# ahmetumutdurmus/zaremba

Measured on NVIDIA H100. Metric: tokens/sec (and valid perplexity) Large-LSTM 1500h at 1/2/4/8 H100 vs ref CPU, higher is better.
Workload: dtype f16 operands, f32 accumulate/state

## Files before the change

zaremba_b200/csrc/common.cuh:

```cuda
#pragma once
#include <cuda_runtime.h>
#include <cuda_fp16.h>
#include <stdint.h>
#include <stdio.h>
#include <atomic>

#include "../../include/zaremba_b200.h"

namespace zrb {

void set_error(const char* fmt, ...);
extern std::atomic<int64_t> g_launches;
extern std::atomic<int> g_live_tc_ctx[64];
inline void count_launch(int n = 1) { g_launches.fetch_add(n, std::memory_order_relaxed); }

#define ZRB_CUDA(call)                                                                   \
    do {                                                                                 \
        cudaError_t e_ = (call);                                                         \
        if (e_ != cudaSuccess) {                                                         \
            zrb::set_error("%s:%d %s -> %s", __FILE__, __LINE__, #call,                  \
                           cudaGetErrorString(e_));                                      \
            return ZRB_E_CUDA;                                                           \
        }                                                                                \
    } while (0)
// ... 105 lines not shown
    for (int i = 0; i < 4; ++i)
        if ((r.v[i] >> 8) >= m.thresh) bits |= 1u << i;
    return bits;
}

__device__ inline uint64_t mask_elem(const MaskSrc& m, uint64_t e) { return m.period ? e % m.period : e; }

__device__ inline float mask_mul1_at(const MaskSrc& m, uint64_t e, uint64_t n_total) {
    if (!m.active) return 1.f;
    uint32_t bits = mask_keep4(m, e >> 2, n_total);
    return ((bits >> (e & 3)) & 1u) ? m.scale : 0.f;
}

__device__ inline void mask_mul4_at(const MaskSrc& m, uint64_t e0, float out[4]) {
    if (!m.active) {
        out[0] = out[1] = out[2] = out[3] = 1.f;
        return;
    }
    const uint32_t sh = (uint32_t)(e0 & 3);
    uint32_t bits = mask_keep4(m, e0 >> 2, ~0ull) >> sh;
    if (sh) bits |= mask_keep4(m, (e0 >> 2) + 1, ~0ull) << (4 - sh);
#pragma unroll
    for (int i = 0; i < 4; ++i) out[i] = ((bits >> i) & 1u) ? m.scale : 0.f;
}

__device__ inline float mask_mul1(const MaskSrc& m, uint64_t e, uint64_t n_total) {
    if (!m.active) return 1.f;
    return mask_mul1_at(m, mask_elem(m, e), n_total);
}

__device__ inline float sigmoidf_(float z) { return 1.f / (1.f + expf(-z)); }

__device__ __forceinline__ float sgd_elem(float p, float g, float lr) { return p - lr * g; }

template <bool RMS>
__device__ __forceinline__ float dyneval_elem(float p, float g, float tg, float r, float lr, float lam, float eps,
                                              float rbar) {
    const float d = __fsub_rn(tg, p);
    const float u = RMS ? __fdiv_rn(g, __fadd_rn(r, eps)) : g;
    const float a = fminf(1.f, RMS ? __fdiv_rn(__fmul_rn(lam, r), rbar) : lam);
    return __fadd_rn(p, __fmaf_rn(a, d, -__fmul_rn(lr, u)));
}

struct DynArgs {
    float lr, lam, eps;
    const float* rbar;
};

__device__ inline float warp_sum(float v) {
#pragma unroll
    for (int o = 16; o > 0; o >>= 1) v += __shfl_xor_sync(0xffffffffu, v, o);
    return v;
}
__device__ inline float warp_max(float v) {
#pragma unroll
    for (int o = 16; o > 0; o >>= 1) v = fmaxf(v, __shfl_xor_sync(0xffffffffu, v, o));
    return v;
}

}
```

zaremba_b200/csrc/engine_tc.cu:

```cuda
#include "engine.h"
#include <stdlib.h>
#include <string.h>

#include "tc_kernels.h"

struct GridBarrier {
    unsigned int* word = nullptr;
    unsigned int base = 0;
    template <typename Launch>
    int claim(int T, int nCTA, cudaStream_t s, Launch&& launch) {
        const unsigned int arrivals = (unsigned int)T * (unsigned int)nCTA;
        if (base > 0xF0000000u - arrivals) {
            ZRB_CUDA(cudaMemsetAsync(word, 0, sizeof(unsigned int), s));
            base = 0;
        }
        ZRB_TRY(launch(word, base));
        base += arrivals;
        return ZRB_OK;
    }
};

struct zrb_tc_state {
    int Xp[ZRB_MAX_LAYERS + 1] = {}, G4p[ZRB_MAX_LAYERS] = {}, Vp = 0;
    int device = 0;
// ... 624 lines not shown
    const RecPlan& bplan = t->bplan[0];
    if (!c->layer_fwd_ok) {
        set_error("zrb_lstm_layer_bwd without a preceding zrb_lstm_layer_fwd");
        return ZRB_E_STATE;
    }
    MaskSrc m = make_mask_src(nullptr, 0, 0, 0, 0.f, 0);
    ZRB_TRY(t->bwd_bar.claim(T, bplan.nCTA, s, [&](unsigned int* word, unsigned int base) {
        return lstm_rec_bwd(bplan, tc_watchdog(c), t->w_img_b[0], t->g_img, dy, c->gates[0], c->cst[0], c->c0s[0], t->dG_h,
                            word, base, T, B, H, G4p, m, m, s, nullptr, db_ih, db_hh, c->resident_flag, ++c->resident_seq, c->dG);
    }));
    const float inv = 1.f / kGradScale;
    if (dx) ZRB_TRY(gemm_f16_tc(t->dG_h, G4p, 0, t->w_ih_h[0], Hp, 1, dx, H, N, H, 4 * H, inv, nullptr, 0, s));
    ZRB_TRY(gemm_f16_tc(t->dG_h, G4p, 1, t->x_h[0], Hp, 1, dw_ih, H, 4 * H, H, N, inv, nullptr, 0, s, nullptr, nullptr, false,
                        t->hprev_h[0], dw_hh, nullptr));
    c->layer_fwd_ok = false;
    return ZRB_OK;
}

int tc_rec_trace(zrb_ctx* c, long long* h_out, int max_entries) {
    if (!c->tc || !c->tc->trace) { set_error("set ZRB_REC_TRACE=1 before creating the context"); return ZRB_E_STATE; }
    int n = 2 * (8 + c->cfg.max_seq * 8);
    if (n > max_entries) n = max_entries;
    ZRB_CUDA(cudaDeviceSynchronize());
    ZRB_CUDA(cudaMemcpy(h_out, c->tc->trace, (size_t)n * sizeof(long long), cudaMemcpyDeviceToHost));
    return n;
}

int tc_update(zrb_ctx* c, const zrb_params* p, const TensorList& tl, float lr, float max_norm, float* norm_out,
              const AvgStep* avg, cudaStream_t s) {
    zrb_tc_state* t = c->tc;
    const int E = c->width[0], V = c->cfg.vocab;
    ZRB_TRY(tc_flush_updates(c, s));
    ProfScope ps(c, ZRB_PROF_CLIP_SGD, s);
    if (!tc_streams_aligned(tl, avg ? avg->a : nullptr)) {
        if (avg) {
            ZRB_TRY(grad_norm(tl, max_norm, c->partials, c->scalars, norm_out, s));
            ZRB_TRY(sgd_avg_apply(tl, avg->a, lr, c->scalars, c->keep_clipped, avg->mu, avg->first, s));
        } else {
            ZRB_TRY(clip_sgd(tl, lr, max_norm, c->partials, c->scalars, norm_out, c->keep_clipped, s));
        }
        c->weights_version++;
        return ZRB_OK;
    }
    const bool rows_only = !c->tied && c->emb_sparse && c->emb_prev_grad == tl.g[0] && c->emb_prev_n > 0;
    const bool gemm_norm = t->wg_ok && t->wg_key == tl.g[tc_matrices(c).fc_w().i];
    TensorList rest = tc_without_matrices(c, tl);
    if (rows_only) rest.n[0] = 0;
    TensorList dense = gemm_norm ? rest : tl;
    if (rows_only) dense.n[0] = 0;
    if (c->tied && gemm_norm) {
        ZRB_TRY(grad_norm(dense, max_norm, c->partials, c->scalars, norm_out, s, true, t->wg_slots));
    } else if (rows_only) {
        ZRB_TRY(embed_first_table(c->emb_prev_ids, c->emb_first, c->emb_prev_n, V, s));
        ZRB_TRY(embed_rows_sumsq(tl.g[0], c->emb_prev_ids, c->emb_first, c->emb_prev_n, E, V,
                                 c->partials + norm_partials_base(), kNormExtra, s));
        ZRB_TRY(grad_norm(dense, max_norm, c->partials, c->scalars, norm_out, s, true, gemm_norm ? t->wg_slots : 0));
        ZRB_TRY(embed_rows_update(tl.p[0], tl.g[0], c->emb_prev_ids, c->emb_first, c->emb_prev_n, E, V, lr, c->scalars,
                                  c->keep_clipped, s));
        if (avg) {
            TensorList e{};
            e.p[0] = tl.p[0]; e.n[0] = tl.n[0]; e.count = 1;
            ZRB_TRY(avg_apply(e, avg->a, avg->mu, avg->first, s));
        }
    } else {
        ZRB_TRY(grad_norm(tl, max_norm, c->partials, c->scalars, norm_out, s));
    }
    const bool lazy = c->lazy_update && t->persistent() && pdl_beside_rec(c);
    if (lazy) {
        t->upd_tl = tl;
        t->upd_lr = lr;
        t->upd_avg_on = avg != nullptr;
        if (avg) t->upd_avg = *avg;
    }
    for (const WeightMatrix& m : tc_matrices(c)) {
        if (lazy && m.item >= 1) t->upd_pending |= 1u << m.item;
        else ZRB_TRY(tc_update_matrix(c, m, tl, lr, avg, false, s));
    }
    if (avg) ZRB_TRY(sgd_avg_apply(rest, avg->a, lr, c->scalars, c->keep_clipped, avg->mu, avg->first, s));
    else ZRB_TRY(sgd_apply(rest, lr, c->scalars, c->keep_clipped, s));
    tc_images_current(c, p);
    return ZRB_OK;
}

int tc_dyneval_update(zrb_ctx* c, const zrb_params* p, const TensorList& tl, float* const* tg, float* const* r,
                      const DynArgs& a, cudaStream_t s) {
    ZRB_TRY(tc_flush_updates(c, s));
    ProfScope ps(c, ZRB_PROF_CLIP_SGD, s);
    if (!tc_streams_aligned(tl, tg, r)) {
        ZRB_TRY(dyneval_apply(tl, tg, r, a, s));
        c->weights_version++;
        return ZRB_OK;
    }
    for (const WeightMatrix& m : tc_matrices(c))
        ZRB_TRY(update_pack_dyn(tl.p[m.i], tl.g[m.i], tg[m.i], r ? r[m.i] : nullptr, m.rows, m.cols, a,
                                tc_images(c, m, {}), s));
    ZRB_TRY(dyneval_apply(tc_without_matrices(c, tl), tg, r, a, s));
    tc_images_current(c, p);
    return ZRB_OK;
}

int tc_swap_average(zrb_ctx* c, const zrb_params* p, const TensorList& tl, float* const* a, cudaStream_t s) {
    ZRB_TRY(tc_flush_updates(c, s));
    ProfScope ps(c, ZRB_PROF_PACK, s);
    if (!tc_streams_aligned(tl, a)) {
        ZRB_TRY(swap_apply(tl, a, s));
        c->weights_version++;
        return ZRB_OK;
    }
    for (const WeightMatrix& m : tc_matrices(c)) ZRB_TRY(swap_pack(tl.p[m.i], a[m.i], m.rows, m.cols, tc_images(c, m, {}), s));
// ... 7 lines not shown
```

zaremba_b200/csrc/kernels.h:

```cpp
#pragma once
#include "common.cuh"

namespace zrb {

int embed_dropout_fwd(const float* W, const int64_t* idx, float* out, __half* out_h, int64_t ld_h,
                      int N, int H, int V, MaskSrc m, MaskSrc em, cudaStream_t s, const float* pend_g = nullptr,
                      float lr = 0.f, const float* scalars = nullptr);
int embed_dropout_bwd(const float* dA, const int64_t* idx, float* dW, int N, int H, int V, MaskSrc m, MaskSrc em,
                      cudaStream_t s);
int lstm_cell_fwd(float* pre, const float* c_prev, float* c_out, float* h_raw, float* y_out, float* h_rec,
                  int B, int H, int64_t elem_off, int64_t n_total, MaskSrc m, MaskSrc rm, cudaStream_t s);
int lstm_cell_bwd(const float* dy_post, const float* dh_rec, float* dc, const float* gates, const float* c_t,
                  const float* c_prev, float* dG, int B, int H, int64_t elem_off, int64_t n_total, MaskSrc m,
                  MaskSrc rm, cudaStream_t s, const float* r = nullptr);
int activation_reg(const float* h, float* r, double* partial, float* out, int T, int B, int H, MaskSrc m, float alpha,
                   float beta, cudaStream_t s);
constexpr int kActRegBlocks = 264;
int dropout_copy(const float* x, float* y, int64_t n, MaskSrc m, cudaStream_t s);
constexpr int kWeightDropBlocks = 264;
int weight_drop(const float* x, float* y, int64_t n, MaskSrc m, float* sumsq, cudaStream_t s);
int add_bias2(float* C, const float* b1, const float* b2, int N, int M, cudaStream_t s);
int add_bias1(float* C, const float* b1, int N, int M, cudaStream_t s);
int colsum(const float* A, float* out, float* out2, int N, int M, cudaStream_t s);
int softmax_nll(const float* scores, const int64_t* y, int N, int V, int B, float* row_loss, float* loss,
                float* dscores, float* tgt_prob, cudaStream_t s, __half* ds_h = nullptr, int64_t ld_s = 0,
                float h_scale = 1.f);
int embed_rows(const float* dA, const int64_t* idx, float* rows, int N, int H, int V, MaskSrc m, MaskSrc em,
               cudaStream_t s);
int embed_scatter_rows(const int64_t* ids, const float* rows, float* dW, int n_rows, int H, int V, int* first,
                       long long* acc, cudaStream_t s, bool add = false, float* sumsq = nullptr, int nblocks = 0);
int embed_zero_rows(float* dW, const int64_t* ids, int n, int H, int V, cudaStream_t s);
int embed_first_table(const int64_t* ids, int* first, int n, int V, cudaStream_t s);
int embed_rows_sumsq(const float* dW, const int64_t* ids, const int* first, int n, int H, int V, float* partial,
                     int nblocks, cudaStream_t s);
int embed_rows_update(float* W, float* dW, const int64_t* ids, const int* first, int n, int H, int V, float lr,
                      const float* scalars, bool write_g, cudaStream_t s);
int dropout_mask_bytes(MaskSrc m, int64_t n, uint8_t* out, cudaStream_t s);

struct TensorList {
    float* p[16];
    float* g[16];
    int64_t n[16];
    int count;
};
constexpr int kNormGemm = 16384;
constexpr int kNormExtra = 1024;
int norm_partials_base();
int grad_norm(const TensorList& tl, float max_norm, float* partials, float* scalars, float* norm_out,
              cudaStream_t s, bool extra_used = false, int n_gemm = 0);
int sgd_apply(const TensorList& tl, float lr, const float* scalars, bool write_g, cudaStream_t s);
int clip_sgd(const TensorList& tl, float lr, float max_norm, float* partials, float* scalars, float* norm_out,
             bool write_g, cudaStream_t s);
int dyneval_apply(const TensorList& tl, float* const* tg, float* const* r, const DynArgs& a, cudaStream_t s);
int sq_accumulate(const TensorList& tl, cudaStream_t s);
constexpr int kStatsPartials = 2048;
int stats_finish(const TensorList& tl, int64_t windows, double* partials, float* rbar, cudaStream_t s);

struct AvgStep {
    float* a[16];
    float mu;
    bool first;
};
int sgd_avg_apply(const TensorList& tl, float* const* a, float lr, const float* scalars, bool write_g, float mu,
                  bool first, cudaStream_t s);
int avg_apply(const TensorList& tl, float* const* a, float mu, bool first, cudaStream_t s);
int swap_apply(const TensorList& tl, float* const* a, cudaStream_t s);

int sample_check(const zrb_sampling* cfg, int B, int V);
int sample_rows(const float* scores, int64_t ld, int B, int V, const zrb_sampling* cfg, uint64_t pos, int64_t* tokens,
                float* logprobs, cudaStream_t s);

struct BeamCand {
    float cand, logp;
    uint32_t flat;
};
struct LayerWidths {
    int h[ZRB_MAX_LAYERS];
};
int beam_check(int B, int K, int V, int eos);
int beam_step(const float* scores, int64_t ld, int B, int K_in, int K, int V, const float* cum_in, const int64_t* tok_in,
              int eos, BeamCand* cands, int64_t* tokens, int32_t* parents, float* cum_out, float* logprobs,
              const zrb_states* src, const zrb_states* dst, int L, const LayerWidths& w, cudaStream_t s);
int beam_backtrack(const int64_t* step_tok, const int32_t* step_par, const float* step_lp, const float* cum, int n_new,
                   int BK, int K, int64_t* tokens, float* logprobs, float* scores, cudaStream_t s);

int gemm_f32(const float* A, const float* B, float* C, int M, int N, int K, int transA, int transB, float alpha,
             float beta, cudaStream_t s);

}
```

zaremba_b200/csrc/optim.cu:

```cuda
#include "kernels.h"

namespace zrb {

constexpr int kNormBlocks = 148 * 8;
constexpr int kThreads = 256;

__device__ __forceinline__ float block_sum(float acc, float* sh) {
    acc = warp_sum(acc);
    if ((threadIdx.x & 31) == 0) sh[threadIdx.x >> 5] = acc;
    __syncthreads();
    float v = 0.f;
    if (threadIdx.x < 32) {
        v = threadIdx.x < kThreads / 32 ? sh[threadIdx.x] : 0.f;
        v = warp_sum(v);
    }
    return v;
}

__device__ __forceinline__ float block_sumsq(const float* __restrict__ g, int64_t n, int bx, int nbx, float* sh) {
    float acc = 0.f;
    const int64_t tid = (int64_t)bx * blockDim.x + threadIdx.x, stride = (int64_t)nbx * blockDim.x;
    if ((((uintptr_t)g) & 15) == 0) {
        const float4* g4 = reinterpret_cast<const float4*>(g);
        const int64_t n4 = n >> 2;
        int64_t i = tid;
        for (; i + 3 * stride < n4; i += 4 * stride) {
            float4 a = __ldcs(g4 + i), b = __ldcs(g4 + i + stride), c = __ldcs(g4 + i + 2 * stride),
                   d = __ldcs(g4 + i + 3 * stride);
            acc += a.x * a.x + a.y * a.y + a.z * a.z + a.w * a.w;
            acc += b.x * b.x + b.y * b.y + b.z * b.z + b.w * b.w;
            acc += c.x * c.x + c.y * c.y + c.z * c.z + c.w * c.w;
            acc += d.x * d.x + d.y * d.y + d.z * d.z + d.w * d.w;
        }
        for (; i < n4; i += stride) {
            float4 a = __ldcs(g4 + i);
            acc += a.x * a.x + a.y * a.y + a.z * a.z + a.w * a.w;
        }
        for (int64_t j = (n4 << 2) + tid; j < n; j += stride) acc += g[j] * g[j];
    } else {
        for (int64_t j = tid; j < n; j += stride) acc += g[j] * g[j];
    }
    return block_sum(acc, sh);
}

struct Runs {
    float* p[16];
    float* g[16];
    int64_t n[16];
};
__global__ void sumsq_kernel(Runs r, float* __restrict__ partials) {
    __shared__ float sh[kThreads / 32];
    float v = block_sumsq(r.g[blockIdx.y], r.n[blockIdx.y], blockIdx.x, gridDim.x, sh);
    if (threadIdx.x == 0) partials[blockIdx.y * gridDim.x + blockIdx.x] = v;
}

__global__ void norm_finalize_kernel(const float* __restrict__ partials, int n, float max_norm,
                                     float* __restrict__ scalars, float* __restrict__ norm_out) {
    __shared__ double sh[32];
    double acc = 0.0;
    int i = threadIdx.x;
    for (; i + 7 * (int)blockDim.x < n; i += 8 * (int)blockDim.x) {
        float v[8];
#pragma unroll
        for (int k = 0; k < 8; ++k) v[k] = partials[i + k * (int)blockDim.x];
#pragma unroll
        for (int k = 0; k < 8; ++k) acc += (double)v[k];
    }
    for (; i < n; i += blockDim.x) acc += (double)partials[i];
    for (int o = 16; o > 0; o >>= 1) acc += __shfl_xor_sync(0xffffffffu, acc, o);
    if ((threadIdx.x & 31) == 0) sh[threadIdx.x >> 5] = acc;
    __syncthreads();
    if (threadIdx.x == 0) {
        double t = 0.0;
        for (int i = 0; i < (int)(blockDim.x >> 5); ++i) t += sh[i];
        float norm = (float)sqrt(t);
        float coef = max_norm / (norm + 1e-6f);
        if (coef > 1.f) coef = 1.f;
        scalars[0] = norm;
        scalars[1] = coef;
        if (norm_out) *norm_out = norm;
    }
}

template <bool WRITE_G>
__global__ void clip_sgd_update_kernel(Runs r, float lr, const float* __restrict__ scalars) {
    float* __restrict__ p = r.p[blockIdx.y];
    float* __restrict__ g = r.g[blockIdx.y];
    const int64_t n = r.n[blockIdx.y];
    const float coef = scalars[1];
    const int64_t tid = (int64_t)blockIdx.x * blockDim.x + threadIdx.x, stride = (int64_t)gridDim.x * blockDim.x;
    if (((((uintptr_t)g) | ((uintptr_t)p)) & 15) == 0) {
        float4* g4 = reinterpret_cast<float4*>(g);
        float4* p4 = reinterpret_cast<float4*>(p);
        const int64_t n4 = n >> 2;
        for (int64_t i = tid; i < n4; i += stride) {
            float4 gv = __ldcs(g4 + i), pv = __ldcs(p4 + i);
            gv.x *= coef; gv.y *= coef; gv.z *= coef; gv.w *= coef;
            pv.x -= lr * gv.x; pv.y -= lr * gv.y; pv.z -= lr * gv.z; pv.w -= lr * gv.w;
            if (WRITE_G) __stcs(g4 + i, gv);
            __stcs(p4 + i, pv);
        }
        for (int64_t j = (n4 << 2) + tid; j < n; j += stride) {
            float gv = g[j] * coef;
            if (WRITE_G) g[j] = gv;
            p[j] -= lr * gv;
        }
    } else {
        for (int64_t j = tid; j < n; j += stride) {
            float gv = g[j] * coef;
            if (WRITE_G) g[j] = gv;
            p[j] -= lr * gv;
        }
    }
}

static int coalesce(const TensorList& tl, Runs* r, int* blocks_per_run) {
    int runs = 0;
    int64_t longest = 0;
    for (int t = 0; t < tl.count; ++t) {
        if (tl.n[t] == 0) continue;
        if (runs && r->p[runs - 1] + r->n[runs - 1] == tl.p[t] && r->g[runs - 1] + r->n[runs - 1] == tl.g[t]) {
            r->n[runs - 1] += tl.n[t];
        } else {
            r->p[runs] = tl.p[t]; r->g[runs] = tl.g[t]; r->n[runs] = tl.n[t];
            ++runs;
        }
    }
    for (int i = runs; i < 16; ++i) { r->p[i] = nullptr; r->g[i] = nullptr; r->n[i] = 0; }
    for (int i = 0; i < runs; ++i) longest = r->n[i] > longest ? r->n[i] : longest;
    int64_t b = (longest / 4 + kThreads - 1) / kThreads;
    if (b < 1) b = 1;
    const int cap = kNormBlocks / (runs > 0 ? runs : 1);
    *blocks_per_run = (int)(b > cap ? cap : b);
    return runs;
}

int norm_partials_base() { return kNormBlocks; }

int grad_norm(const TensorList& tl, float max_norm, float* partials, float* scalars, float* norm_out,
              cudaStream_t s, bool extra_used, int n_gemm) {
    Runs r;
    int bpr = 1;
    const int runs = coalesce(tl, &r, &bpr);
    ZRB_CUDA(cudaMemsetAsync(partials, 0, (kNormBlocks + (extra_used ? 0 : kNormExtra)) * sizeof(float), s));
    if (runs) {
        sumsq_kernel<<<dim3(bpr, runs), kThreads, 0, s>>>(r, partials);
        ZRB_KERNEL_CHECK();
    }
    norm_finalize_kernel<<<1, 1024, 0, s>>>(partials, kNormBlocks + kNormExtra + n_gemm, max_norm, scalars, norm_out);
    ZRB_KERNEL_CHECK();
    return ZRB_OK;
}

int sgd_apply(const TensorList& tl, float lr, const float* scalars, bool write_g, cudaStream_t s) {
    Runs r;
    int bpr = 1;
    const int runs = coalesce(tl, &r, &bpr);
    if (!runs) return ZRB_OK;
    int64_t longest = 0;
    for (int i = 0; i < runs; ++i) longest = r.n[i] > longest ? r.n[i] : longest;
    int64_t b = (longest / 4 + kThreads - 1) / kThreads;
    const int bx = (int)(b < 1 ? 1 : (b > kNormBlocks ? kNormBlocks : b)) * 2;
    if (write_g) clip_sgd_update_kernel<true><<<dim3(bx, runs), kThreads, 0, s>>>(r, lr, scalars);
    else clip_sgd_update_kernel<false><<<dim3(bx, runs), kThreads, 0, s>>>(r, lr, scalars);
    ZRB_KERNEL_CHECK();
    return ZRB_OK;
}

int clip_sgd(const TensorList& tl, float lr, float max_norm, float* partials, float* scalars, float* norm_out,
             bool write_g, cudaStream_t s) {
    ZRB_TRY(grad_norm(tl, max_norm, partials, scalars, norm_out, s));
    return sgd_apply(tl, lr, scalars, write_g, s);
}

struct DynRuns {
    float* p[16];
    const float* g[16];
    const float* tg[16];
    const float* r[16];
    int64_t n[16];
};

static int dyn_runs(const TensorList& tl, float* const* tg, float* const* r, DynRuns* d, int* bx, int cap) {
    int k = 0;
    int64_t longest = 0;
    for (int t = 0; t < tl.count; ++t) {
        if (tl.n[t] == 0) continue;
        d->p[k] = tl.p[t]; d->g[k] = tl.g[t]; d->n[k] = tl.n[t];
        d->tg[k] = tg ? tg[t] : nullptr;
        d->r[k] = r ? r[t] : nullptr;
        longest = tl.n[t] > longest ? tl.n[t] : longest;
        ++k;
    }
    int64_t b = (longest / 4 + kThreads - 1) / kThreads;
    if (b < 1) b = 1;
    const int c = cap / (k > 0 ? k : 1);
    *bx = (int)(b > c ? c : b);
    return k;
}

template <bool RMS>
// ... 116 lines not shown
```

zaremba_b200/csrc/pointwise.cu:

```cuda
#include "kernels.h"

namespace zrb {

template <bool PENDING>
__global__ void embed_dropout_fwd_kernel(const float* __restrict__ W, const int64_t* __restrict__ idx,
                                         float* __restrict__ out, __half* __restrict__ out_h, int64_t ld_h, int N,
                                         int H, int V, MaskSrc m, MaskSrc em, const float* __restrict__ pend_g, float lr,
                                         const float* __restrict__ scalars) {
    int n = blockIdx.x;
    if (n >= N) return;
    int64_t row = idx[n];
    if (row < 0 || row >= V) row = 0;
    const float* src = W + row * (int64_t)H;
    int groups = (H + 3) >> 2;
    uint64_t n_total = (uint64_t)N * H;
    float coef = 0.f;
    if constexpr (PENDING) coef = scalars[1];
    const float se = em.active ? mask_mul1_at(em, (uint64_t)row, (uint64_t)V) : 1.f;
    for (int g = threadIdx.x; g < groups; g += blockDim.x) {
        int j0 = g << 2;
        uint64_t e0 = (uint64_t)n * H + j0;
        float v[4];
#pragma unroll
        for (int i = 0; i < 4; ++i) {
// ... 513 lines not shown
        if (id < 0 || id >= V || first[id] != n) continue;
        for (int j = threadIdx.x; j < H; j += blockDim.x) {
            const float old = dW[id * (int64_t)H + j];
            const float e = (float)((double)acc[(int64_t)n * H + j] * (1.0 / 1099511627776.0));
            const float nw = old + e;
            dW[id * (int64_t)H + j] = nw;
            ss += (double)nw * nw - (double)old * old;
        }
    }
    if (!sumsq) return;
#pragma unroll
    for (int o = 16; o > 0; o >>= 1) ss += __shfl_xor_sync(0xffffffffu, ss, o);
    if ((threadIdx.x & 31) == 0) sh[threadIdx.x >> 5] = ss;
    __syncthreads();
    if (threadIdx.x == 0) {
        double t = 0.0;
        for (int i = 0; i < (int)(blockDim.x >> 5); ++i) t += sh[i];
        sumsq[blockIdx.x] = (float)t;
    }
}
int embed_scatter_rows(const int64_t* ids, const float* rows, float* dW, int n_rows, int H, int V, int* first,
                       long long* acc, cudaStream_t s, bool add, float* sumsq, int nblocks) {
    if (!n_rows) return ZRB_OK;
    ZRB_CUDA(cudaMemsetAsync(first, 0x7f, (size_t)V * sizeof(int), s));
    ZRB_CUDA(cudaMemsetAsync(acc, 0, (size_t)n_rows * H * sizeof(long long), s));
    embed_first_kernel<<<cdiv(n_rows, 256), 256, 0, s>>>(ids, first, n_rows, V);
    ZRB_KERNEL_CHECK();
    embed_accum_kernel<<<n_rows, 256, 0, s>>>(ids, rows, first, acc, n_rows, H, V);
    ZRB_KERNEL_CHECK();
    if (add) embed_finish_add_kernel<<<sumsq ? nblocks : n_rows, 256, 0, s>>>(ids, first, acc, dW, n_rows, H, V, sumsq);
    else embed_finish_kernel<<<n_rows, 256, 0, s>>>(ids, first, acc, dW, n_rows, H, V);
    ZRB_KERNEL_CHECK();
    return ZRB_OK;
}

__global__ void embed_zero_rows_kernel(float* __restrict__ dW, const int64_t* __restrict__ ids, int n, int H, int V) {
    const int64_t id = ids[blockIdx.x];
    if (id < 0 || id >= V) return;
    for (int j = threadIdx.x; j < H; j += blockDim.x) dW[id * (int64_t)H + j] = 0.f;
}
int embed_zero_rows(float* dW, const int64_t* ids, int n, int H, int V, cudaStream_t s) {
    if (!n) return ZRB_OK;
    embed_zero_rows_kernel<<<n, 256, 0, s>>>(dW, ids, n, H, V);
    ZRB_KERNEL_CHECK();
    return ZRB_OK;
}
int embed_first_table(const int64_t* ids, int* first, int n, int V, cudaStream_t s) {
    ZRB_CUDA(cudaMemsetAsync(first, 0x7f, (size_t)V * sizeof(int), s));
    if (!n) return ZRB_OK;
    embed_first_kernel<<<cdiv(n, 256), 256, 0, s>>>(ids, first, n, V);
    ZRB_KERNEL_CHECK();
    return ZRB_OK;
}
__global__ void embed_rows_sumsq_kernel(const float* __restrict__ dW, const int64_t* __restrict__ ids,
                                        const int* __restrict__ first, int n, int H, int V, float* __restrict__ partial) {
    __shared__ float sh[8];
    float acc = 0.f;
    for (int t = blockIdx.x; t < n; t += gridDim.x) {
        const int64_t id = ids[t];
        if (id < 0 || id >= V || first[id] != t) continue;
        for (int j = threadIdx.x; j < H; j += blockDim.x) {
            float v = dW[id * (int64_t)H + j];
            acc += v * v;
        }
    }
    acc = warp_sum(acc);
    if ((threadIdx.x & 31) == 0) sh[threadIdx.x >> 5] = acc;
    __syncthreads();
    if (threadIdx.x == 0) {
        float t = 0.f;
        for (int i = 0; i < (int)(blockDim.x >> 5); ++i) t += sh[i];
        partial[blockIdx.x] = t;
    }
}
int embed_rows_sumsq(const float* dW, const int64_t* ids, const int* first, int n, int H, int V, float* partial,
                     int nblocks, cudaStream_t s) {
    embed_rows_sumsq_kernel<<<nblocks, 256, 0, s>>>(dW, ids, first, n, H, V, partial);
    ZRB_KERNEL_CHECK();
    return ZRB_OK;
}
__global__ void embed_rows_update_kernel(float* __restrict__ W, float* __restrict__ dW, const int64_t* __restrict__ ids,
                                         const int* __restrict__ first, int n, int H, int V, float lr,
                                         const float* __restrict__ scalars, bool write_g) {
    const int t = blockIdx.x;
    const int64_t id = ids[t];
    if (id < 0 || id >= V || first[id] != t) return;
    const float coef = scalars[1];
    for (int j = threadIdx.x; j < H; j += blockDim.x) {
        float g = dW[id * (int64_t)H + j] * coef;
        if (write_g) dW[id * (int64_t)H + j] = g;
        W[id * (int64_t)H + j] -= lr * g;
    }
}
int embed_rows_update(float* W, float* dW, const int64_t* ids, const int* first, int n, int H, int V, float lr,
                      const float* scalars, bool write_g, cudaStream_t s) {
    if (!n) return ZRB_OK;
    embed_rows_update_kernel<<<n, 256, 0, s>>>(W, dW, ids, first, n, H, V, lr, scalars, write_g);
    ZRB_KERNEL_CHECK();
    return ZRB_OK;
}

__global__ void dropout_mask_kernel(MaskSrc m, int64_t n, uint8_t* __restrict__ out) {
    int64_t g = (int64_t)blockIdx.x * blockDim.x + threadIdx.x;
    if (4 * g >= n) return;
    uint32_t bits = m.active ? mask_keep4(m, (uint64_t)g, (uint64_t)n) : 0xFu;
    for (int i = 0; i < 4; ++i)
        if (4 * g + i < n) out[4 * g + i] = (bits >> i) & 1u;
}
int dropout_mask_bytes(MaskSrc m, int64_t n, uint8_t* out, cudaStream_t s) {
    if (!n) return ZRB_OK;
    dropout_mask_kernel<<<cdiv((n + 3) / 4, 256), 256, 0, s>>>(m, n, out);
    ZRB_KERNEL_CHECK();
    return ZRB_OK;
}

}
```

zaremba_b200/csrc/update_tile.cuh:

```cuda
#pragma once
#include "tc_kernels.h"

namespace zrb {

struct PackSpec {
    __half* row_img;
    int64_t ld;
    __half* fwd_img;
    int fU, fG, fKc, fKS;
    __half* bwd_img;
    int bUC, bG, bKc, bS;
    int write_g;
    int pdl;
};

__device__ __forceinline__ void pdl_prologue(const PackSpec& sp) {
    if (sp.pdl && threadIdx.x == 0) asm volatile("griddepcontrol.launch_dependents;" ::: "memory");
}
__device__ __forceinline__ void pdl_epilogue(const PackSpec& sp) {
    if (sp.pdl && blockIdx.x == 0 && threadIdx.x == 0) asm volatile("griddepcontrol.wait;" ::: "memory");
}

template <int VEC> struct VecT;
template <> struct VecT<4> { using type = float4; };
template <> struct VecT<2> { using type = float2; };
template <> struct VecT<1> { using type = float; };

template <int VEC>
__device__ __forceinline__ void load_vec(const float* p, float (&v)[VEC]) {
    typename VecT<VEC>::type t = __ldcs(reinterpret_cast<const typename VecT<VEC>::type*>(p));
    const float* f = reinterpret_cast<const float*>(&t);
#pragma unroll
    for (int i = 0; i < VEC; ++i) v[i] = f[i];
}
__device__ __forceinline__ void st_v2(__half* dst, uint32_t a, uint32_t b) {
    asm volatile("st.global.v2.b32 [%0], {%1, %2};" ::"l"(dst), "r"(a), "r"(b));
}
__device__ __forceinline__ void st_v4(__half* dst, const uint4& v) {
    asm volatile("st.global.v4.b32 [%0], {%1, %2, %3, %4};" ::"l"(dst), "r"(v.x), "r"(v.y), "r"(v.z), "r"(v.w));
}

template <int VEC>
__device__ __forceinline__ void pack_row(const float (&v)[VEC], uint32_t (&w)[(VEC + 1) / 2]) {
    if constexpr (VEC == 1) {
        w[0] = __half_as_ushort(__float2half_rn(v[0]));
    } else {
#pragma unroll
        for (int k = 0; k < VEC / 2; ++k) {
            const __half2 h = __floats2half2_rn(v[2 * k], v[2 * k + 1]);
            w[k] = *reinterpret_cast<const uint32_t*>(&h);
        }
    }
}
template <int VEC>
__device__ __forceinline__ void store_halves(__half* dst, const uint32_t (&w)[(VEC + 1) / 2]) {
    if constexpr (VEC == 4) st_v2(dst, w[0], w[1]);
    else if constexpr (VEC == 2) *reinterpret_cast<uint32_t*>(dst) = w[0];
    else *reinterpret_cast<unsigned short*>(dst) = (unsigned short)w[0];
}

template <int VEC>
__device__ __forceinline__ void store_vec(float* p, const float (&v)[VEC]) {
    typename VecT<VEC>::type t;
    float* f = reinterpret_cast<float*>(&t);
#pragma unroll
    for (int i = 0; i < VEC; ++i) f[i] = v[i];
    __stcs(reinterpret_cast<typename VecT<VEC>::type*>(p), t);
}

constexpr int kTileRows = 8;
constexpr int kUpdThreads = 128;

struct NoTileRule {
    template <int VEC> struct Tile {};
    template <int VEC> __device__ __forceinline__ void load(int64_t, int, Tile<VEC>&) const {}
    template <int VEC> __device__ __forceinline__ void finish(int, const float (&)[VEC], Tile<VEC>&) const {}
    template <int VEC> __device__ __forceinline__ void store(int64_t, int, const Tile<VEC>&) const {}
};

struct SgdRule : NoTileRule {
    float lr;
    const float* scalars;
    float coef;
    static constexpr bool kMayWriteG = true;
    static constexpr int kWhhMinBlocks = 5;
    __device__ __forceinline__ void init() { coef = scalars[1]; }
    template <int VEC>
    __device__ __forceinline__ void apply(int64_t, float (&pv)[VEC], float (&gv)[VEC]) const {
#pragma unroll
        for (int x = 0; x < VEC; ++x) { gv[x] *= coef; pv[x] = sgd_elem(pv[x], gv[x], lr); }
    }
};

template <int VEC, class Rule>
__device__ __forceinline__ void tile_update(const float* __restrict__ p, const float* __restrict__ g, int64_t off,
                                            int stride, int n, const Rule& rule, float (&pv)[kTileRows][VEC],
                                            float (&gv)[kTileRows][VEC], typename Rule::template Tile<VEC>& tile) {
#pragma unroll
    for (int e = 0; e < kTileRows; ++e) {
        if (e < n) {
            load_vec<VEC>(g + off + (int64_t)e * stride, gv[e]);
            load_vec<VEC>(p + off + (int64_t)e * stride, pv[e]);
            rule.template load<VEC>(off + (int64_t)e * stride, e, tile);
        }
    }
#pragma unroll
    for (int e = 0; e < kTileRows; ++e) {
        if (e < n) {
            rule.template apply<VEC>(off + (int64_t)e * stride, pv[e], gv[e]);
            rule.template finish<VEC>(e, pv[e], tile);
        }
    }
}

template <int VEC, class Rule>
__device__ __forceinline__ void tile_store(float* __restrict__ p, float* __restrict__ g, int64_t off, int stride, int n,
                                           bool write_g, const float (&pv)[kTileRows][VEC],
                                           const float (&gv)[kTileRows][VEC], const Rule& rule,
                                           const typename Rule::template Tile<VEC>& tile) {
#pragma unroll
    for (int e = 0; e < kTileRows; ++e) {
        if (e < n) {
            if (write_g) store_vec<VEC>(g + off + (int64_t)e * stride, gv[e]);
            store_vec<VEC>(p + off + (int64_t)e * stride, pv[e]);
            rule.template store<VEC>(off + (int64_t)e * stride, e, tile);
        }
    }
}


template <int VEC, class Rule>
__global__ void __launch_bounds__(kUpdThreads) update_pack_kernel(float* __restrict__ p, float* __restrict__ g, int rows,
                                                                  int cols, int col_tiles, Rule rule, PackSpec sp) {
    pdl_prologue(sp);
    rule.init();
    const unsigned rg = blockIdx.x / (unsigned)col_tiles, ct = blockIdx.x - rg * col_tiles;
    const int c = (ct * blockDim.x + threadIdx.x) * VEC;
    const int r0 = rg * kTileRows, n = min(kTileRows, rows - r0);
    if (c < cols) {
        const int64_t off = (int64_t)r0 * cols + c;
        float pv[kTileRows][VEC], gv[kTileRows][VEC];
        typename Rule::template Tile<VEC> tile;
        tile_update<VEC>(p, g, off, cols, n, rule, pv, gv, tile);
        tile_store<VEC>(p, g, off, cols, n, Rule::kMayWriteG && sp.write_g, pv, gv, rule, tile);
        if (sp.row_img) {
#pragma unroll
            for (int e = 0; e < kTileRows; ++e) {
                if (e < n) {
                    uint32_t w[(VEC + 1) / 2];
                    pack_row<VEC>(pv[e], w);
                    store_halves<VEC>(sp.row_img + (int64_t)(r0 + e) * sp.ld + c, w);
                }
            }
        }
    }
    pdl_epilogue(sp);
}

template <int VEC, class Rule>
__global__ void __launch_bounds__(kUpdThreads, Rule::kWhhMinBlocks) update_pack_whh_kernel(float* __restrict__ p, float* __restrict__ g,
                                                                      int H, int col_tiles, Rule rule, PackSpec sp) {
    pdl_prologue(sp);
    rule.init();
    const int lane = threadIdx.x & 31, q = lane & 3;
    const unsigned jb = blockIdx.x / (unsigned)col_tiles, ct = blockIdx.x - jb * col_tiles;
    const int c = ((ct * (blockDim.x >> 5) + (threadIdx.x >> 5)) * 8 + (lane >> 2)) * VEC;
    const int j0 = jb * kTileRows, n = min(kTileRows, H - j0);
    uint32_t hw[kTileRows][(VEC + 1) / 2];
    if (c < H) {
        const int64_t off = ((int64_t)q * H + j0) * H + c;
        float pv[kTileRows][VEC], gv[kTileRows][VEC];
        typename Rule::template Tile<VEC> tile;
        tile_update<VEC>(p, g, off, H, n, rule, pv, gv, tile);
#pragma unroll
        for (int e = 0; e < kTileRows; ++e) {
            if (e < n) {
                pack_row<VEC>(pv[e], hw[e]);
            } else {
#pragma unroll
                for (int k = 0; k < (VEC + 1) / 2; ++k) hw[e][k] = 0;
            }
        }
        tile_store<VEC>(p, g, off, H, n, Rule::kMayWriteG && sp.write_g, pv, gv, rule, tile);
        if (sp.row_img) {
#pragma unroll
            for (int e = 0; e < kTileRows; ++e)
                if (e < n) store_halves<VEC>(sp.row_img + (int64_t)(q * H + j0 + e) * sp.ld + c, hw[e]);
        }
        if (sp.fwd_img) {
            const unsigned kc = (unsigned)c >> 3, kq = kc / (unsigned)sp.fKc, kcl = kc - kq * sp.fKc;
            unsigned cluster = (unsigned)j0 / (unsigned)sp.fU, u = j0 - cluster * sp.fU;
#pragma unroll
            for (int e = 0; e < kTileRows; ++e) {
                if (e < n) {
                    const unsigned row = 4 * u + q, cta = cluster * sp.fKS + kq;
                    store_halves<VEC>(sp.fwd_img + ((int64_t)(cta * sp.fKc + kcl) * sp.fG + (row >> 3)) * 64 +
                                          (row & 7) * 8 + (c & 7), hw[e]);
                }
                if (++u == (unsigned)sp.fU) { u = 0; ++cluster; }
            }
        }
    } else {
#pragma unroll
        for (int e = 0; e < kTileRows; ++e)
#pragma unroll
            for (int k = 0; k < (VEC + 1) / 2; ++k) hw[e][k] = 0;
    }
    if (sp.bwd_img) {
        uint4 v[VEC];
#pragma unroll
        for (int x = 0; x < VEC; ++x) {
            uint32_t w[4];
#pragma unroll
            for (int m = 0; m < 4; ++m)
                w[m] = VEC == 1 ? hw[2 * m][0] | (hw[2 * m + 1][0] << 16)
                                : __byte_perm(hw[2 * m][x >> 1], hw[2 * m + 1][x >> 1], (x & 1) ? 0x7632 : 0x5410);
            v[x] = make_uint4(w[0], w[1], w[2], w[3]);
        }
        const unsigned rank = q * sp.bS + jb / (unsigned)sp.bKc, kcl = jb - (jb / sp.bKc) * sp.bKc;
        __half* base = sp.bwd_img + (int64_t)kcl * sp.bG * 64;
        auto put = [&](int unit, const uint4& val) {
            if (unit < H) {
                const unsigned cl = (unsigned)unit / (unsigned)sp.bUC, u = unit - cl * sp.bUC;
                st_v4(base + (int64_t)((cl * 4 * sp.bS + rank) * sp.bKc) * sp.bG * 64 + (u >> 3) * 64 + (u & 7) * 8, val);
            }
        };
        if constexpr (VEC == 1) {
            put(c, v[0]);
        } else {
            const bool lower = ((lane >> 2) & 1) == 0;
            const int a = lower ? c : c - VEC;
            uint4 recv[VEC / 2];
#pragma unroll
            for (int m = 0; m < VEC / 2; ++m) {
                const uint4 s = lower ? v[2 * m + 1] : v[2 * m];
                recv[m] = make_uint4(__shfl_xor_sync(0xffffffffu, s.x, 4), __shfl_xor_sync(0xffffffffu, s.y, 4),
                                     __shfl_xor_sync(0xffffffffu, s.z, 4), __shfl_xor_sync(0xffffffffu, s.w, 4));
            }
#pragma unroll
            for (int i = 0; i < VEC; ++i) {
                if (lower) put(a + 2 * i, i < VEC / 2 ? v[2 * i] : recv[i - VEC / 2]);
                else put(a + 2 * i + 1, i < VEC / 2 ? recv[i] : v[2 * (i - VEC / 2) + 1]);
            }
        }
    }
    pdl_epilogue(sp);
}

template <int VEC, class Rule>
static int update_pack_launch(float* p, float* g, int rows, int cols, const Rule& rule, const PackSpec& sp, bool whh,
                              cudaStream_t s) {
    const int cv = cols / VEC;
    int threads = kUpdThreads, col_tiles;
    if (whh) {
        col_tiles = (cv + 8 * (threads / 32) - 1) / (8 * (threads / 32));
    } else {
        threads = min(kUpdThreads, (cv + 31) / 32 * 32);
        col_tiles = (cv + threads - 1) / threads;
    }
    const dim3 grid((unsigned)(((rows / (whh ? 4 : 1)) + kTileRows - 1) / kTileRows * col_tiles));
    if (sp.pdl) {
        cudaLaunchConfig_t cfg = {};
        cfg.gridDim = grid; cfg.blockDim = dim3(threads); cfg.dynamicSmemBytes = 12 * 1024; cfg.stream = s;
        cudaLaunchAttribute at[1];
        at[0].id = cudaLaunchAttributeProgrammaticStreamSerialization;
        at[0].val.programmaticStreamSerializationAllowed = 1;
        cfg.attrs = at; cfg.numAttrs = 1;
        if (whh) ZRB_CUDA(cudaLaunchKernelEx(&cfg, update_pack_whh_kernel<VEC, Rule>, p, g, cols, col_tiles, rule, sp));
        else ZRB_CUDA(cudaLaunchKernelEx(&cfg, update_pack_kernel<VEC, Rule>, p, g, rows, cols, col_tiles, rule, sp));
        count_launch();
        return ZRB_OK;
    }
    if (whh) update_pack_whh_kernel<VEC, Rule><<<grid, threads, 0, s>>>(p, g, cols, col_tiles, rule, sp);
    else update_pack_kernel<VEC, Rule><<<grid, threads, 0, s>>>(p, g, rows, cols, col_tiles, rule, sp);
    ZRB_KERNEL_CHECK();
    return ZRB_OK;
}

template <class Rule>
static int update_pack_rule(float* p, float* g, int rows, int cols, const Rule& rule, uintptr_t align,
                            const WeightImages& img, bool write_g, cudaStream_t s, bool pdl) {
    const RecPlan *fp = img.fplan, *bp = img.bplan;
    PackSpec sp;
    sp.write_g = write_g ? 1 : 0;
    sp.pdl = pdl ? 1 : 0;
    sp.row_img = img.row; sp.ld = img.ld;
    sp.fwd_img = img.fwd; sp.fKS = fp ? fp->KS : 1; sp.fU = fp ? fp->KS * fp->U : 1; sp.fG = fp ? fp->G : 1;
    sp.fKc = fp ? fp->KcS : 1;
    sp.bwd_img = img.bwd; sp.bS = bp ? bp->KS : 1; sp.bUC = bp ? 4 * bp->KS * bp->U : 4; sp.bG = bp ? bp->G : 1;
    sp.bKc = bp ? bp->KcS : 1;
    const bool whh = (img.fwd || img.bwd) && rows == 4 * cols;
    const uintptr_t all = ((uintptr_t)p) | ((uintptr_t)g) | align;
    const bool al16 = (all & 15) == 0, al8 = (all & 7) == 0;
    if (cols % 4 == 0 && al16) return update_pack_launch<4>(p, g, rows, cols, rule, sp, whh, s);
    if (cols % 2 == 0 && al8) return update_pack_launch<2>(p, g, rows, cols, rule, sp, whh, s);
// ... 5 lines not shown
```

Baseline: 390,100.

## Fuse norm partials, vectorize embed row update, stage W_hh packing via shared memory

Merges the memset, dense sumsq kernel and embedding-row sumsq kernel into one launch that also zeroes unused partial slots, removing two launches per step. Vectorizes the sparse embedding SGD update with float4 when aligned. Reworks the W_hh pack epilogue to stage fp16 rows in shared memory so forward-image writes become 16-byte stores and backward-image transposition reads from shared memory instead of shuffles. This adds shared-memory use per block, which may affect occupancy.

Result: no change. 393,800 (median of 6 runs) (+1.0%).

```diff
diff --git a/zaremba_b200/csrc/common.cuh b/zaremba_b200/csrc/common.cuh
--- a/zaremba_b200/csrc/common.cuh
+++ b/zaremba_b200/csrc/common.cuh
@@ -181,6 +181,26 @@
     for (int o = 16; o > 0; o >>= 1) v += __shfl_xor_sync(0xffffffffu, v, o);
     return v;
 }
+__device__ inline float embed_rows_sumsq_block(const float* __restrict__ dW, const int64_t* __restrict__ ids,
+                                               const int* __restrict__ first, int n, int H, int V, int bx, int nbx,
+                                               float* sh) {
+    float acc = 0.f;
+    for (int t = bx; t < n; t += nbx) {
+        const int64_t id = ids[t];
+        if (id < 0 || id >= V || first[id] != t) continue;
+        for (int j = threadIdx.x; j < H; j += blockDim.x) {
+            float v = dW[id * (int64_t)H + j];
+            acc += v * v;
+        }
+    }
+    acc = warp_sum(acc);
+    if ((threadIdx.x & 31) == 0) sh[threadIdx.x >> 5] = acc;
+    __syncthreads();
+    float t = 0.f;
+    if (threadIdx.x == 0)
+        for (int i = 0; i < (int)(blockDim.x >> 5); ++i) t += sh[i];
+    return t;
+}
 __device__ inline float warp_max(float v) {
 #pragma unroll
     for (int o = 16; o > 0; o >>= 1) v = fmaxf(v, __shfl_xor_sync(0xffffffffu, v, o));
diff --git a/zaremba_b200/csrc/engine_tc.cu b/zaremba_b200/csrc/engine_tc.cu
--- a/zaremba_b200/csrc/engine_tc.cu
+++ b/zaremba_b200/csrc/engine_tc.cu
@@ -700,9 +700,9 @@
         ZRB_TRY(grad_norm(dense, max_norm, c->partials, c->scalars, norm_out, s, true, t->wg_slots));
     } else if (rows_only) {
         ZRB_TRY(embed_first_table(c->emb_prev_ids, c->emb_first, c->emb_prev_n, V, s));
-        ZRB_TRY(embed_rows_sumsq(tl.g[0], c->emb_prev_ids, c->emb_first, c->emb_prev_n, E, V,
-                                 c->partials + norm_partials_base(), kNormExtra, s));
-        ZRB_TRY(grad_norm(dense, max_norm, c->partials, c->scalars, norm_out, s, true, gemm_norm ? t->wg_slots : 0));
+        const EmbedRowsNorm rows = {tl.g[0], c->emb_prev_ids, c->emb_first, c->emb_prev_n, E, V};
+        ZRB_TRY(grad_norm(dense, max_norm, c->partials, c->scalars, norm_out, s, true, gemm_norm ? t->wg_slots : 0,
+                          &rows));
         ZRB_TRY(embed_rows_update(tl.p[0], tl.g[0], c->emb_prev_ids, c->emb_first, c->emb_prev_n, E, V, lr, c->scalars,
                                   c->keep_clipped, s));
         if (avg) {
diff --git a/zaremba_b200/csrc/kernels.h b/zaremba_b200/csrc/kernels.h
--- a/zaremba_b200/csrc/kernels.h
+++ b/zaremba_b200/csrc/kernels.h
@@ -31,8 +31,6 @@
                        long long* acc, cudaStream_t s, bool add = false, float* sumsq = nullptr, int nblocks = 0);
 int embed_zero_rows(float* dW, const int64_t* ids, int n, int H, int V, cudaStream_t s);
 int embed_first_table(const int64_t* ids, int* first, int n, int V, cudaStream_t s);
-int embed_rows_sumsq(const float* dW, const int64_t* ids, const int* first, int n, int H, int V, float* partial,
-                     int nblocks, cudaStream_t s);
 int embed_rows_update(float* W, float* dW, const int64_t* ids, const int* first, int n, int H, int V, float lr,
                       const float* scalars, bool write_g, cudaStream_t s);
 int dropout_mask_bytes(MaskSrc m, int64_t n, uint8_t* out, cudaStream_t s);
@@ -46,8 +44,14 @@
 constexpr int kNormGemm = 16384;
 constexpr int kNormExtra = 1024;
 int norm_partials_base();
+struct EmbedRowsNorm {
+    const float* dW;
+    const int64_t* ids;
+    const int* first;
+    int n, H, V;
+};
 int grad_norm(const TensorList& tl, float max_norm, float* partials, float* scalars, float* norm_out,
-              cudaStream_t s, bool extra_used = false, int n_gemm = 0);
+              cudaStream_t s, bool extra_used = false, int n_gemm = 0, const EmbedRowsNorm* rows = nullptr);
 int sgd_apply(const TensorList& tl, float lr, const float* scalars, bool write_g, cudaStream_t s);
 int clip_sgd(const TensorList& tl, float lr, float max_norm, float* partials, float* scalars, float* norm_out,
              bool write_g, cudaStream_t s);
diff --git a/zaremba_b200/csrc/optim.cu b/zaremba_b200/csrc/optim.cu
--- a/zaremba_b200/csrc/optim.cu
+++ b/zaremba_b200/csrc/optim.cu
@@ -48,11 +48,6 @@
     float* g[16];
     int64_t n[16];
 };
-__global__ void sumsq_kernel(Runs r, float* __restrict__ partials) {
-    __shared__ float sh[kThreads / 32];
-    float v = block_sumsq(r.g[blockIdx.y], r.n[blockIdx.y], blockIdx.x, gridDim.x, sh);
-    if (threadIdx.x == 0) partials[blockIdx.y * gridDim.x + blockIdx.x] = v;
-}
 
 __global__ void norm_finalize_kernel(const float* __restrict__ partials, int n, float max_norm,
                                      float* __restrict__ scalars, float* __restrict__ norm_out) {
@@ -137,16 +132,39 @@
 
 int norm_partials_base() { return kNormBlocks; }
 
+__global__ void norm_partials_kernel(Runs r, int bpr, int nsum, EmbedRowsNorm e, int zero_end,
+                                     float* __restrict__ partials) {
+    __shared__ float sh[kThreads / 32];
+    const int b = blockIdx.x;
+    if (b < nsum) {
+        const int y = b / bpr, x = b - y * bpr;
+        const float v = block_sumsq(r.g[y], r.n[y], x, bpr, sh);
+        if (threadIdx.x == 0) partials[b] = v;
+        return;
+    }
+    const int ne = e.dW ? kNormExtra : 0;
+    if (b < nsum + ne) {
+        const int k = b - nsum;
+        const float v = embed_rows_sumsq_block(e.dW, e.ids, e.first, e.n, e.H, e.V, k, kNormExtra, sh);
+        if (threadIdx.x == 0) partials[kNormBlocks + k] = v;
+        return;
+    }
+    const int i = nsum + (b - nsum - ne) * kThreads + threadIdx.x;
+    if (i < zero_end) partials[i] = 0.f;
+}
+
 int grad_norm(const TensorList& tl, float max_norm, float* partials, float* scalars, float* norm_out,
-              cudaStream_t s, bool extra_used, int n_gemm) {
+              cudaStream_t s, bool extra_used, int n_gemm, const EmbedRowsNorm* rows) {
     Runs r;
     int bpr = 1;
     const int runs = coalesce(tl, &r, &bpr);
-    ZRB_CUDA(cudaMemsetAsync(partials, 0, (kNormBlocks + (extra_used ? 0 : kNormExtra)) * sizeof(float), s));
-    if (runs) {
-        sumsq_kernel<<<dim3(bpr, runs), kThreads, 0, s>>>(r, partials);
-        ZRB_KERNEL_CHECK();
-    }
+    EmbedRowsNorm e = {};
+    if (rows && rows->n > 0) e = *rows;
+    const int nsum = runs * bpr, ne = e.dW ? kNormExtra : 0;
+    const int zero_end = kNormBlocks + (extra_used || e.dW ? 0 : kNormExtra);
+    const int nzero = (zero_end - nsum + kThreads - 1) / kThreads;
+    norm_partials_kernel<<<nsum + ne + nzero, kThreads, 0, s>>>(r, bpr, nsum, e, zero_end, partials);
+    ZRB_KERNEL_CHECK();
     norm_finalize_kernel<<<1, 1024, 0, s>>>(partials, kNormBlocks + kNormExtra + n_gemm, max_norm, scalars, norm_out);
     ZRB_KERNEL_CHECK();
     return ZRB_OK;
diff --git a/zaremba_b200/csrc/pointwise.cu b/zaremba_b200/csrc/pointwise.cu
--- a/zaremba_b200/csrc/pointwise.cu
+++ b/zaremba_b200/csrc/pointwise.cu
@@ -589,33 +589,6 @@
     ZRB_KERNEL_CHECK();
     return ZRB_OK;
 }
-__global__ void embed_rows_sumsq_kernel(const float* __restrict__ dW, const int64_t* __restrict__ ids,
-                                        const int* __restrict__ first, int n, int H, int V, float* __restrict__ partial) {
-    __shared__ float sh[8];
-    float acc = 0.f;
-    for (int t = blockIdx.x; t < n; t += gridDim.x) {
-        const int64_t id = ids[t];
-        if (id < 0 || id >= V || first[id] != t) continue;
-        for (int j = threadIdx.x; j < H; j += blockDim.x) {
-            float v = dW[id * (int64_t)H + j];
-            acc += v * v;
-        }
-    }
-    acc = warp_sum(acc);
-    if ((threadIdx.x & 31) == 0) sh[threadIdx.x >> 5] = acc;
-    __syncthreads();
-    if (threadIdx.x == 0) {
-        float t = 0.f;
-        for (int i = 0; i < (int)(blockDim.x >> 5); ++i) t += sh[i];
-        partial[blockIdx.x] = t;
-    }
-}
-int embed_rows_sumsq(const float* dW, const int64_t* ids, const int* first, int n, int H, int V, float* partial,
-                     int nblocks, cudaStream_t s) {
-    embed_rows_sumsq_kernel<<<nblocks, 256, 0, s>>>(dW, ids, first, n, H, V, partial);
-    ZRB_KERNEL_CHECK();
-    return ZRB_OK;
-}
 __global__ void embed_rows_update_kernel(float* __restrict__ W, float* __restrict__ dW, const int64_t* __restrict__ ids,
                                          const int* __restrict__ first, int n, int H, int V, float lr,
                                          const float* __restrict__ scalars, bool write_g) {
@@ -623,6 +596,18 @@
     const int64_t id = ids[t];
     if (id < 0 || id >= V || first[id] != t) return;
     const float coef = scalars[1];
+    if (((H & 3) | ((((uintptr_t)W) | ((uintptr_t)dW)) & 15)) == 0) {
+        float4* w4 = reinterpret_cast<float4*>(W + id * (int64_t)H);
+        float4* g4 = reinterpret_cast<float4*>(dW + id * (int64_t)H);
+        for (int j = threadIdx.x; j < (H >> 2); j += blockDim.x) {
+            float4 g = g4[j], w = w4[j];
+            g.x *= coef; g.y *= coef; g.z *= coef; g.w *= coef;
+            if (write_g) g4[j] = g;
+            w.x -= lr * g.x; w.y -= lr * g.y; w.z -= lr * g.z; w.w -= lr * g.w;
+            w4[j] = w;
+        }
+        return;
+    }
     for (int j = threadIdx.x; j < H; j += blockDim.x) {
         float g = dW[id * (int64_t)H + j] * coef;
         if (write_g) dW[id * (int64_t)H + j] = g;
diff --git a/zaremba_b200/csrc/update_tile.cuh b/zaremba_b200/csrc/update_tile.cuh
--- a/zaremba_b200/csrc/update_tile.cuh
+++ b/zaremba_b200/csrc/update_tile.cuh
@@ -55,6 +55,13 @@
 template <int VEC>
 __device__ __forceinline__ void store_halves(__half* dst, const uint32_t (&w)[(VEC + 1) / 2]) {
     if constexpr (VEC == 4) st_v2(dst, w[0], w[1]);
+    else if constexpr (VEC == 2) *reinterpret_cast<uint32_t*>(dst) = w[0];
+    else *reinterpret_cast<unsigned short*>(dst) = (unsigned short)w[0];
+}
+
+template <int VEC>
+__device__ __forceinline__ void stage_halves(__half* dst, const uint32_t (&w)[(VEC + 1) / 2]) {
+    if constexpr (VEC == 4) *reinterpret_cast<uint2*>(dst) = make_uint2(w[0], w[1]);
     else if constexpr (VEC == 2) *reinterpret_cast<uint32_t*>(dst) = w[0];
     else *reinterpret_cast<unsigned short*>(dst) = (unsigned short)w[0];
 }
@@ -160,13 +167,16 @@
 template <int VEC, class Rule>
 __global__ void __launch_bounds__(kUpdThreads, Rule::kWhhMinBlocks) update_pack_whh_kernel(float* __restrict__ p, float* __restrict__ g,
                                                                       int H, int col_tiles, Rule rule, PackSpec sp) {
+    constexpr int kCols = 8 * VEC;
+    constexpr int kPitch = VEC == 1 ? 8 : kCols + 8;
+    __shared__ __align__(16) __half stage[kUpdThreads / 32][4 * kTileRows][kPitch];
     pdl_prologue(sp);
     rule.init();
-    const int lane = threadIdx.x & 31, q = lane & 3;
+    const int lane = threadIdx.x & 31, q = lane & 3, warp = threadIdx.x >> 5;
     const unsigned jb = blockIdx.x / (unsigned)col_tiles, ct = blockIdx.x - jb * col_tiles;
-    const int c = ((ct * (blockDim.x >> 5) + (threadIdx.x >> 5)) * 8 + (lane >> 2)) * VEC;
+    const int c0 = (ct * (blockDim.x >> 5) + warp) * kCols, cl = (lane >> 2) * VEC, c = c0 + cl;
     const int j0 = jb * kTileRows, n = min(kTileRows, H - j0);
-    uint32_t hw[kTileRows][(VEC + 1) / 2];
+    __half (*st)[kPitch] = stage[warp];
     if (c < H) {
         const int64_t off = ((int64_t)q * H + j0) * H + c;
         float pv[kTileRows][VEC], gv[kTileRows][VEC];
@@ -174,73 +184,65 @@
         tile_update<VEC>(p, g, off, H, n, rule, pv, gv, tile);
 #pragma unroll
         for (int e = 0; e < kTileRows; ++e) {
-            if (e < n) {
-                pack_row<VEC>(pv[e], hw[e]);
-            } else {
-#pragma unroll
-                for (int k = 0; k < (VEC + 1) / 2; ++k) hw[e][k] = 0;
-            }
+            uint32_t w[(VEC + 1) / 2] = {};
+            if (e < n) pack_row<VEC>(pv[e], w);
+            stage_halves<VEC>(&st[4 * e + q][cl], w);
         }
         tile_store<VEC>(p, g, off, H, n, Rule::kMayWriteG && sp.write_g, pv, gv, rule, tile);
         if (sp.row_img) {
 #pragma unroll
-            for (int e = 0; e < kTileRows; ++e)
-                if (e < n) store_halves<VEC>(sp.row_img + (int64_t)(q * H + j0 + e) * sp.ld + c, hw[e]);
-        }
-        if (sp.fwd_img) {
-            const unsigned kc = (unsigned)c >> 3, kq = kc / (unsigned)sp.fKc, kcl = kc - kq * sp.fKc;
-            unsigned cluster = (unsigned)j0 / (unsigned)sp.fU, u = j0 - cluster * sp.fU;
-#pragma unroll
             for (int e = 0; e < kTileRows; ++e) {
                 if (e < n) {
-                    const unsigned row = 4 * u + q, cta = cluster * sp.fKS + kq;
-                    store_halves<VEC>(sp.fwd_img + ((int64_t)(cta * sp.fKc + kcl) * sp.fG + (row >> 3)) * 64 +
-                                          (row & 7) * 8 + (c & 7), hw[e]);
+                    uint32_t w[(VEC + 1) / 2];
+                    pack_row<VEC>(pv[e], w);
+                    store_halves<VEC>(sp.row_img + (int64_t)(q * H + j0 + e) * sp.ld + c, w);
                 }
-                if (++u == (unsigned)sp.fU) { u = 0; ++cluster; }
             }
         }
     } else {
 #pragma unroll
-        for (int e = 0; e < kTileRows; ++e)
-#pragma unroll
-            for (int k = 0; k < (VEC + 1) / 2; ++k) hw[e][k] = 0;
+        for (int e = 0; e < kTileRows; ++e) {
+            const uint32_t w[(VEC + 1) / 2] = {};
+            stage_halves<VEC>(&st[4 * e + q][cl], w);
+        }
+    }
+    __syncwarp();
+    if (sp.fwd_img) {
+        const int e = lane >> 2;
+        if (e < n) {
+            const unsigned j = j0 + e, cluster = j / (unsigned)sp.fU, u = j - cluster * sp.fU, row = 4 * u + q;
+#pragma unroll
+            for (int i = 0; i < VEC; ++i) {
+                const int k0 = c0 + 8 * i;
+                if (k0 < H) {
+                    const unsigned kc = (unsigned)k0 >> 3, kq = kc / (unsigned)sp.fKc, kcl = kc - kq * sp.fKc;
+                    const unsigned cta = cluster * sp.fKS + kq;
+                    __half* dst = sp.fwd_img + ((int64_t)(cta * sp.fKc + kcl) * sp.fG + (row >> 3)) * 64 + (row & 7) * 8;
+                    const __half* src = &st[lane][8 * i];
+                    if (k0 + 8 <= H) {
+                        st_v4(dst, *reinterpret_cast<const uint4*>(src));
+                    } else {
+                        for (int k = 0; k < H - k0; ++k) dst[k] = src[k];
+                    }
+                }
+            }
+        }
     }
     if (sp.bwd_img) {
-        uint4 v[VEC];
-#pragma unroll
-        for (int x = 0; x < VEC; ++x) {
-            uint32_t w[4];
-#pragma unroll
-            for (int m = 0; m < 4; ++m)
-                w[m] = VEC == 1 ? hw[2 * m][0] | (hw[2 * m + 1][0] << 16)
-                                : __byte_perm(hw[2 * m][x >> 1], hw[2 * m + 1][x >> 1], (x & 1) ? 0x7632 : 0x5410);
-            v[x] = make_uint4(w[0], w[1], w[2], w[3]);
-        }
-        const unsigned rank = q * sp.bS + jb / (unsigned)sp.bKc, kcl = jb - (jb / sp.bKc) * sp.bKc;
+        const unsigned short* s16 = reinterpret_cast<const unsigned short*>(&st[0][0]);
+        const unsigned kb = jb / (unsigned)sp.bKc, kcl = jb - kb * sp.bKc;
         __half* base = sp.bwd_img + (int64_t)kcl * sp.bG * 64;
-        auto put = [&](int unit, const uint4& val) {
+#pragma unroll
+        for (int i = 0; i < VEC; ++i) {
+            const int k = 32 * i + lane, gq = k / kCols, ul = k - gq * kCols, unit = c0 + ul;
             if (unit < H) {
-                const unsigned cl = (unsigned)unit / (unsigned)sp.bUC, u = unit - cl * sp.bUC;
-                st_v4(base + (int64_t)((cl * 4 * sp.bS + rank) * sp.bKc) * sp.bG * 64 + (u >> 3) * 64 + (u & 7) * 8, val);
-            }
-        };
-        if constexpr (VEC == 1) {
-            put(c, v[0]);
-        } else {
-            const bool lower = ((lane >> 2) & 1) == 0;
-            const int a = lower ? c : c - VEC;
-            uint4 recv[VEC / 2];
-#pragma unroll
-            for (int m = 0; m < VEC / 2; ++m) {
-                const uint4 s = lower ? v[2 * m + 1] : v[2 * m];
-                recv[m] = make_uint4(__shfl_xor_sync(0xffffffffu, s.x, 4), __shfl_xor_sync(0xffffffffu, s.y, 4),
-                                     __shfl_xor_sync(0xffffffffu, s.z, 4), __shfl_xor_sync(0xffffffffu, s.w, 4));
-            }
-#pragma unroll
-            for (int i = 0; i < VEC; ++i) {
-                if (lower) put(a + 2 * i, i < VEC / 2 ? v[2 * i] : recv[i - VEC / 2]);
-                else put(a + 2 * i + 1, i < VEC / 2 ? recv[i] : v[2 * (i - VEC / 2) + 1]);
+                uint32_t w[4];
+#pragma unroll
+                for (int m = 0; m < 4; ++m)
+                    w[m] = (uint32_t)s16[(8 * m + gq) * kPitch + ul] | ((uint32_t)s16[(8 * m + 4 + gq) * kPitch + ul] << 16);
+                const unsigned rank = gq * sp.bS + kb, ucl = (unsigned)unit / (unsigned)sp.bUC, u = unit - ucl * sp.bUC;
+                st_v4(base + (int64_t)((ucl * 4 * sp.bS + rank) * sp.bKc) * sp.bG * 64 + (u >> 3) * 64 + (u & 7) * 8,
+                      make_uint4(w[0], w[1], w[2], w[3]));
             }
         }
     }
```
